# Megvii-CSG/MegReader

Hardware: AMD Instinct MI355X
Metric: training images/sec, CRNN-CTC 32x128 crops, batch 256 per GPU (higher is better)
Workload: dtype bf16; 1 GPU; CRNN + 1D-CTC training step (BASELINE.json configs[1]): 32x128 crops, T=33, C=38, Adam; global_batch=256, per_gpu_batch=256, parallelism=dp1, launch=hipGraph replay

## Files before the change

megreader_amd/csrc/igemm_core.h:

```cpp
#pragma once
#include "common.h"
#include <type_traits>

namespace mr {

struct ConvGeom {
  int Hg, Wg, Cg, ldg;
  int Hm, Wm;
  int R, S, sh, sw, ph, pw, dh, dw;
  int mode;
};

__device__ __forceinline__ bool conv_src(const ConvGeom& g, int hm, int wm, int r, int s, int& hi, int& wi) {
  if (g.mode == 1) {
    hi = hm * g.sh - g.ph + r * g.dh;
    wi = wm * g.sw - g.pw + s * g.dw;
  } else {
    int hn = hm + g.ph - r * g.dh;
    int wn = wm + g.pw - s * g.dw;
    if (hn < 0 || wn < 0) return false;
    if (g.sh == 1 && g.sw == 1) {
      hi = hn;
      wi = wn;
    } else {
      hi = hn / g.sh;
      wi = wn / g.sw;
      if (hi * g.sh != hn || wi * g.sw != wn) return false;
    }
  }
  return (unsigned)hi < (unsigned)g.Hg && (unsigned)wi < (unsigned)g.Wg;
}

template <typename T> struct Mma;
template <> struct Mma<bf16_t> {
  typedef bf16x8 Frag;
  static __device__ __forceinline__ void run(f32x4& acc, const Frag& a, const Frag& b) {
    acc = __builtin_amdgcn_mfma_f32_16x16x32_bf16(a, b, acc, 0, 0, 0);
  }
};
template <> struct Mma<float> {
  typedef f32x4 Frag;
  static __device__ __forceinline__ void run(f32x4& acc, const Frag& a, const Frag& b) {
#pragma unroll
    for (int j = 0; j < 4; ++j) acc = __builtin_amdgcn_mfma_f32_16x16x4f32(a[j], b[j], acc, 0, 0, 0);
  }
};

struct NtArgs {
  const void* A;
  const void* B;
  int M, N, K;
  long long lda;
  int ldb;
  const void* zero;
  int m_begin = 0;
  int ksplit = 1;
  void* ws = nullptr;
  int tile_rows = 0;
};
constexpr int NT_SPLIT_TICKETS = 4096;

__device__ __forceinline__ uint4 ldg16(const void* p) { return *(const uint4*)p; }

template <typename Epi> struct EpiHasStats { static constexpr bool value = false; };
template <typename Epi> struct EpiIsPool { static constexpr bool value = false; };
__device__ __forceinline__ float row16_sum(float v) {
#define MR_ROW_ROR(V, N) __builtin_bit_cast(float, __builtin_amdgcn_update_dpp(0, __builtin_bit_cast(int, V), 0x120 + (N), 0xf, 0xf, false))
  v += MR_ROW_ROR(v, 8);
  v += MR_ROW_ROR(v, 4);
  v += MR_ROW_ROR(v, 2);
  v += MR_ROW_ROR(v, 1);
#undef MR_ROW_ROR
  return v;
}
template <typename T, int CNT> struct EpiColStats {
  float s[4 * CNT], q[4 * CNT];
  __device__ __forceinline__ void init() {
#pragma unroll
    for (int e = 0; e < 4 * CNT; ++e) s[e] = q[e] = 0.f;
  }
  template <typename Epi> __device__ __forceinline__ void add(const Epi& epi, int m, int n, const f32x4* v) {
    if (m >= epi.M) return;
    if constexpr (Epi::kBnb) {
      const long long row = (long long)m * epi.ldc + n;
#pragma unroll
      for (int i = 0; i < CNT; ++i)
#pragma unroll
        for (int j = 0; j < 4; ++j) {
          const int c = 4 * i + j;
          if (n + c < epi.N) {
            float t = v[i][j];
            if (epi.addend) t += to_f32(epi.addend[row + c]);
            t = to_f32(from_f32<T>(t));
            if (epi.bnb_y && !(to_f32(epi.bnb_y[row + c]) > 0.f)) t = 0.f;
            s[c] += t;
            q[c] += t * to_f32(epi.bnb_x[row + c]);
          }
        }
    } else {
#pragma unroll
      for (int i = 0; i < CNT; ++i)
#pragma unroll
        for (int j = 0; j < 4; ++j) {
          float t = v[i][j];
          if (epi.bias && n + 4 * i + j < epi.N) t += epi.bias[n + 4 * i + j];
          t = to_f32(from_f32<T>(t));
          s[4 * i + j] += t;
          q[4 * i + j] += t * t;
        }
    }
  }
  template <typename Epi> __device__ __forceinline__ double q_out(const Epi& epi, int c, float sv, float qv) const {
    if constexpr (Epi::kBnb) return ((double)qv - (double)epi.bnb_mean[c] * (double)sv) * (double)epi.bnb_rstd[c];
    else return (double)qv;
  }
  template <typename Epi> __device__ __forceinline__ void flush(const Epi& epi, int n, int l15) {
#pragma unroll
    for (int e = 0; e < 4 * CNT; ++e) {
      s[e] = row16_sum(s[e]);
      q[e] = row16_sum(q[e]);
    }
    double* dst = epi.stats + (size_t)(blockIdx.x % epi.stats_ncopy) * 2 * epi.N;
    if constexpr (CNT == 4) {
      float sv = s[0], qv = q[0];
#pragma unroll
      for (int e = 1; e < 16; ++e) {
        sv = l15 == e ? s[e] : sv;
        qv = l15 == e ? q[e] : qv;
      }
      if (n + l15 < epi.N) {
        atomicAdd(dst + n + l15, (double)sv);
        atomicAdd(dst + epi.N + n + l15, q_out(epi, n + l15, sv, qv));
      }
    } else if constexpr (CNT == 2) {
      const int c = l15 & 7;
      float sv = s[0], qv = q[0];
#pragma unroll
      for (int e = 1; e < 8; ++e) {
        sv = c == e ? s[e] : sv;
        qv = c == e ? q[e] : qv;
      }
      if (n + c < epi.N) {
        if (l15 < 8) atomicAdd(dst + n + c, (double)sv);
        else atomicAdd(dst + epi.N + n + c, q_out(epi, n + c, sv, qv));
      }
    } else {
      if (l15 != 0) return;
#pragma unroll
      for (int e = 0; e < 4 * CNT; ++e)
        if (n + e < epi.N) {
          atomicAdd(dst + n + e, (double)s[e]);
          atomicAdd(dst + epi.N + n + e, q_out(epi, n + e, s[e], q[e]));
        }
    }
  }
};


template <typename T, int BM, int BN, int AMODE, typename Epi>
__device__ __forceinline__ void igemm_nt_body(const NtArgs& a, const ConvGeom& g, const Epi& epi) {
  constexpr int VEC = VecOf<T>::N;
  constexpr int BK = 8 * VEC;
  constexpr int AI = BM / 32, BI = BN / 32;
  constexpr int WTM = BM / 2, WTN = BN / 2, TM = WTM / 16, TN = WTN / 16;
  typedef typename Mma<T>::Frag Frag;

  __shared__ uint4 smem[8 * (BM + BN)];
  uint4* sA = smem;
  uint4* sB = smem + 8 * BM;

  const int tid = threadIdx.x;
  const int tiles_n = (a.N + BN - 1) / BN;
  const int tile_n = blockIdx.x % tiles_n, tile_m = blockIdx.x / tiles_n;
  const int m0 = tile_m * BM, n0 = tile_n * BN;
  const int kc = tid & 7, r0 = tid >> 3;

  const T* __restrict__ A = (const T*)a.A;
  const T* __restrict__ B = (const T*)a.B;

  long long a_off[AI];
  int a_h[AI], a_w[AI];
  unsigned a_mask[AI];
  bool a_ok[AI];
#pragma unroll
  for (int i = 0; i < AI; ++i) {
    const int m = m0 + r0 + 32 * i;
    a_ok[i] = m < a.M;
    a_mask[i] = 0;
    if (AMODE == 0) {
      a_off[i] = (long long)m * a.lda;
      a_h[i] = a_w[i] = 0;
    } else {
      const int wm = m % g.Wm;
      const int t = m / g.Wm;
      const int hm = t % g.Hm;
      const int ni = t / g.Hm;
      a_off[i] = (long long)ni * g.Hg * g.Wg * g.ldg;
      a_h[i] = hm;
      a_w[i] = wm;
      if (AMODE == 2) {
        const int bh = g.mode == 1 ? hm * g.sh - g.ph : hm + g.ph;
        const int bw = g.mode == 1 ? wm * g.sw - g.pw : wm + g.pw;
        a_off[i] += ((long long)bh * g.Wg + bw) * g.ldg;
        if (a_ok[i]) {
          unsigned msk = 0;
          for (int r = 0; r < g.R; ++r)
            for (int s2 = 0; s2 < g.S; ++s2) {
              int hi, wi;
              if (conv_src(g, hm, wm, r, s2, hi, wi)) msk |= 1u << (r * g.S + s2);
            }
          a_mask[i] = msk;
        }
      }
    }
  }
  long long b_off[BI];
  bool b_ok[BI];
#pragma unroll
  for (int i = 0; i < BI; ++i) {
    const int n = n0 + r0 + 32 * i;
    b_ok[i] = n < a.N;
    b_off[i] = (long long)n * a.ldb;
  }

  uint4 ra[AI], rb[BI];
  int f_tap = 0, f_r = 0, f_s = 0, f_c = kc * VEC;
  if (AMODE == 2) {
    while (f_c >= g.Cg) {
      f_c -= g.Cg;
      ++f_tap;
      if (++f_s == g.S) { f_s = 0; ++f_r; }
    }
  }
  const int taps = g.R * g.S;
  auto load_tiles = [&](int k0) {
    const int k = k0 + kc * VEC;
    const bool kok = k < a.K;
    int r = 0, s = 0, c = k;
    if (AMODE == 1) {
      const int tap = k / g.Cg;
      c = k - tap * g.Cg;
      r = tap / g.S;
      s = tap - r * g.S;
    }
    if (AMODE == 2) {
      const int toff = (f_r * g.dh * g.Wg + f_s * g.dw) * g.ldg;
      const long long koff = (long long)(g.mode == 1 ? toff : -toff) + f_c;
      const bool tok = f_tap < taps;
#pragma unroll
      for (int i = 0; i < AI; ++i) {
        uint4 v = make_uint4(0, 0, 0, 0);
        if (tok && ((a_mask[i] >> f_tap) & 1u)) v = ldg16(A + a_off[i] + koff);
        ra[i] = v;
      }
      f_c += BK;
      while (f_c >= g.Cg) {
        f_c -= g.Cg;
        ++f_tap;
        if (++f_s == g.S) { f_s = 0; ++f_r; }
      }
    } else {
#pragma unroll
      for (int i = 0; i < AI; ++i) {
        uint4 v = make_uint4(0, 0, 0, 0);
        if (a_ok[i] && kok) {
          if (AMODE == 0) {
            v = ldg16(A + a_off[i] + k);
          } else {
            int hi, wi;
            if (conv_src(g, a_h[i], a_w[i], r, s, hi, wi))
              v = ldg16(A + a_off[i] + ((long long)hi * g.Wg + wi) * g.ldg + c);
          }
        }
        ra[i] = v;
      }
    }
#pragma unroll
    for (int i = 0; i < BI; ++i) {
      uint4 v = make_uint4(0, 0, 0, 0);
      if (b_ok[i] && kok) v = ldg16(B + b_off[i] + k);
      rb[i] = v;
    }
  };

  const int wave = tid >> 6, lane = tid & 63;
  const int wm_ = wave & 1, wn_ = wave >> 1;
  const int l15 = lane & 15, lg = lane >> 4;

  f32x4 acc[TN][TM];
#pragma unroll
  for (int i = 0; i < TN; ++i)
#pragma unroll
    for (int j = 0; j < TM; ++j) acc[i][j] = (f32x4){0.f, 0.f, 0.f, 0.f};
  constexpr bool WIDE = sizeof(T) == 4;
  double tot[WIDE ? TN : 1][WIDE ? TM : 1][4];
  if constexpr (WIDE) {
#pragma unroll
    for (int i = 0; i < TN; ++i)
#pragma unroll
      for (int j = 0; j < TM; ++j)
#pragma unroll
        for (int e = 0; e < 4; ++e) tot[i][j][e] = 0.0;
  }

  load_tiles(0);
  for (int k0 = 0; k0 < a.K; k0 += BK) {
#pragma unroll
    for (int i = 0; i < AI; ++i) sA[kc * BM + ((r0 + 32 * i) ^ kc)] = ra[i];
#pragma unroll
// ... 356 lines not shown
#pragma unroll
    for (int i = 0; i < BI; ++i) {
      const bool ok = b_ok[i] && (k_exact || k0 + b_kc[i] < a.K);
      glds16_buf(rsB, ok, b_ptr[i] + k0, ESH, sB + (wave * BI + i) * 64);
    }
  };

  const int wm_ = wave & 1, wn_ = wave >> 1;
  const int l15 = lane & 15, lg = lane >> 4;
  const int xsw = (l15 >> 1) & 7;
  int fa_off[TM][2], fb_off[TN][2];
#pragma unroll
  for (int j = 0; j < TM; ++j) {
    const int r = wm_ * WTM + j * 16 + l15;
    fa_off[j][0] = r * 8 + (lg ^ xsw);
    fa_off[j][1] = r * 8 + ((lg ^ xsw) ^ 4);
  }
#pragma unroll
  for (int i = 0; i < TN; ++i) {
    const int r = wn_ * WTN + i * 16 + l15;
    fb_off[i][0] = BM * 8 + r * 8 + (lg ^ xsw);
    fb_off[i][1] = BM * 8 + r * 8 + ((lg ^ xsw) ^ 4);
  }

  f32x4 acc[TN][TM];
#pragma unroll
  for (int i = 0; i < TN; ++i)
#pragma unroll
    for (int j = 0; j < TM; ++j) acc[i][j] = (f32x4){0.f, 0.f, 0.f, 0.f};
  constexpr bool WIDE = sizeof(T) == 4;
  double tot[WIDE ? TN : 1][WIDE ? TM : 1][4];
  if constexpr (WIDE) {
#pragma unroll
    for (int i = 0; i < TN; ++i)
#pragma unroll
      for (int j = 0; j < TM; ++j)
#pragma unroll
        for (int e = 0; e < 4; ++e) tot[i][j][e] = 0.0;
  }

  auto compute = [&](const uint4* st) {
#pragma unroll
    for (int ks = 0; ks < 2; ++ks) {
      Frag fa[TM], fb[TN];
#pragma unroll
      for (int j = 0; j < TM; ++j) fa[j] = *(const Frag*)&st[fa_off[j][ks]];
#pragma unroll
      for (int i = 0; i < TN; ++i) fb[i] = *(const Frag*)&st[fb_off[i][ks]];
#pragma unroll
      for (int i = 0; i < TN; ++i)
#pragma unroll
        for (int j = 0; j < TM; ++j) Mma<T>::run(acc[i][j], fb[i], fa[j]);
    }
    if constexpr (WIDE) {
#pragma unroll
      for (int i = 0; i < TN; ++i)
#pragma unroll
        for (int j = 0; j < TM; ++j) {
#pragma unroll
          for (int e = 0; e < 4; ++e) tot[i][j][e] += (double)acc[i][j][e];
          acc[i][j] = (f32x4){0.f, 0.f, 0.f, 0.f};
        }
    }
  };

  const int nk_all = (a.K + BK - 1) / BK;
  int nk = nk_all, kb = 0;
  if (a.ksplit > 1) {
    const int per = (nk_all + a.ksplit - 1) / a.ksplit;
    const int first = (int)blockIdx.y * per;
    kb = first * BK;
    nk = min(per, nk_all - first);
    if (AMODE == 2) {
      s_tap = kb / g.Cg;
      s_c0 = kb - s_tap * g.Cg;
      s_r = s_tap / g.S;
      s_s = s_tap - s_r * g.S;
    }
  }
  if constexpr (NST == 2) {
    uint4* st0 = smem;
    uint4* st1 = smem + TILE_VECS;
    if (nk > 0) stage(st0, kb);
    int t = 0;
    for (; t + 1 < nk; t += 2) {
      __syncthreads();
      stage(st1, kb + (t + 1) * BK);
      compute(st0);
      __syncthreads();
      if (t + 2 < nk) stage(st0, kb + (t + 2) * BK);
      compute(st1);
    }
    if (t < nk) {
      __syncthreads();
      compute(st0);
    }
  } else {
    constexpr int LPS = AI + BI;
    static_assert((NST - 2) * LPS <= 63, "vmcnt is a 6-bit counter");
#pragma unroll
    for (int u = 0; u < NST - 1; ++u)
      if (u < nk) stage(smem + u * TILE_VECS, kb + u * BK);
    for (int t0 = 0; t0 < nk; t0 += NST) {
#pragma unroll
      for (int u = 0; u < NST; ++u) {
        const int t = t0 + u;
        if (t < nk) {
          const int younger = min(NST - 2, nk - 1 - t);
          if (younger >= 2 && NST >= 4) asm volatile("s_waitcnt vmcnt(%0)\n\ts_barrier" ::"n"(2 * LPS) : "memory");
          else if (younger == 1) asm volatile("s_waitcnt vmcnt(%0)\n\ts_barrier" ::"n"(LPS) : "memory");
          else asm volatile("s_waitcnt vmcnt(0)\n\ts_barrier" ::: "memory");
          if (t + NST - 1 < nk) stage(smem + ((u + NST - 1) % NST) * TILE_VECS, kb + (t + NST - 1) * BK);
          compute(smem + u * TILE_VECS);
        }
      }
    }
  }

  if constexpr (!WIDE) {
    if (a.ksplit > 1) {
      typedef __attribute__((ext_vector_type(4))) unsigned u32x4s;
      const int tile_lin = tile_m * tiles_n + tile_n;
      const rsrc_t rs = __builtin_amdgcn_make_buffer_rsrc((char*)a.ws + NT_SPLIT_TICKETS * 4, (short)0, 0x7fffffff, 0x00020000);
      constexpr int SLAB = BM * BN * 4;
      const int so = (tile_lin * a.ksplit + (int)blockIdx.y) * SLAB;
#pragma unroll
      for (int i = 0; i < TN; ++i)
#pragma unroll
        for (int j = 0; j < TM; ++j)
          __builtin_amdgcn_raw_buffer_store_b128(__builtin_bit_cast(u32x4s, acc[i][j]), rs, tid * 16, so + (i * TM + j) * 4096, 16);
      asm volatile("s_waitcnt vmcnt(0)" ::: "memory");
      __syncthreads();
      volatile int* bc = (volatile int*)smem;
      int* tk = (int*)a.ws + (tile_lin % NT_SPLIT_TICKETS);
      if (tid == 0) *bc = __hip_atomic_fetch_add(tk, 1, __ATOMIC_RELAXED, __HIP_MEMORY_SCOPE_AGENT);
      __syncthreads();
      if (*bc != a.ksplit - 1) return;
      if (tid == 0) __hip_atomic_store(tk, 0, __ATOMIC_RELAXED, __HIP_MEMORY_SCOPE_AGENT);
#pragma unroll
      for (int i = 0; i < TN; ++i)
#pragma unroll
        for (int j = 0; j < TM; ++j) acc[i][j] = (f32x4){0.f, 0.f, 0.f, 0.f};
      for (int sp = 0; sp < a.ksplit; ++sp) {
        const int sj = (tile_lin * a.ksplit + sp) * SLAB;
#pragma unroll
        for (int i = 0; i < TN; ++i)
#pragma unroll
          for (int j = 0; j < TM; ++j)
            acc[i][j] += __builtin_bit_cast(f32x4, __builtin_amdgcn_raw_buffer_load_b128(rs, tid * 16, sj + (i * TM + j) * 4096, 16));
      }
    }
  }

  EpiColStats<T, TN> cst;
  bool with_stats = false;
  if constexpr (EpiHasStats<Epi>::value) with_stats = epi.stats != nullptr;
  if (with_stats) cst.init();
#pragma unroll
  for (int j = 0; j < TM; ++j) {
    f32x4 run[TN];
#pragma unroll
    for (int i = 0; i < TN; ++i) {
      if constexpr (WIDE) run[i] = (f32x4){(float)tot[i][j][0], (float)tot[i][j][1], (float)tot[i][j][2], (float)tot[i][j][3]};
      else run[i] = acc[i][j];
    }
    if constexpr (EpiHasStats<Epi>::value)
      if (with_stats) cst.add(epi, m0 + wm_ * WTM + j * 16 + l15, n0 + wn_ * WTN + lg * (4 * TN), run);
    epi.template store_run<TN>(m0 + wm_ * WTM + j * 16 + l15, n0 + wn_ * WTN + lg * (4 * TN), run);
  }
  if constexpr (EpiHasStats<Epi>::value)
    if (with_stats) cst.flush(epi, n0 + wn_ * WTN + lg * (4 * TN), l15);
}

template <typename T, int WM, int WN, int TM, int TN, int AMODE, typename Epi>
__global__ __launch_bounds__(64 * WM * WN) void igemm_nt_big_kernel(NtArgs a, ConvGeom g, Epi epi) {
  constexpr int VEC = VecOf<T>::N;
  constexpr int BK = 8 * VEC;
  constexpr int NW = WM * WN;
  constexpr int WTM = TM * 16, WTN = TN * 16, BM = WM * WTM, BN = WN * WTN;
  constexpr int AG = BM / 8, BG = BN / 8;
  constexpr int AI = (AG + NW - 1) / NW, BI = (BG + NW - 1) / NW;
  constexpr int TILE_VECS = (BM + BN) * 8;
  typedef typename Mma<T>::Frag Frag;
  static_assert(AMODE == 0 || AMODE == 2, "big-tile kernel: dense or fast conv gather only");

  extern __shared__ uint4 smem_big[];
  uint4* smem = smem_big;

  const int tid = threadIdx.x;
  const int wave = __builtin_amdgcn_readfirstlane(tid >> 6);
  const int lane = tid & 63;
  const int trows = a.tile_rows > 0 ? a.tile_rows : BM;
  const int tiles_n = (a.N + BN - 1) / BN, tiles_m = (a.M - a.m_begin + trows - 1) / trows;
  const int xcd = blockIdx.x & 7, slot = blockIdx.x >> 3;
  const int tile_m = (slot / tiles_n) * 8 + xcd, tile_n = slot % tiles_n;
  if (tile_m >= tiles_m) return;
  const int m0 = a.m_begin + tile_m * trows, n0 = tile_n * BN;
  const int lrow = lane >> 3, lpc = lane & 7;

  const T* __restrict__ A = (const T*)a.A;
  const T* __restrict__ B = (const T*)a.B;
  (void)a.zero;
  constexpr int ESH = sizeof(T) == 2 ? 1 : 2;
  const rsrc_t rsA = make_rsrc(A), rsB = make_rsrc(B);

  auto kc_of = [&](int gi) { return (lpc ^ (((gi * 8 + lrow) >> 1) & 7)) * VEC; };
  int a_off[AI];
  unsigned a_mask[AI];
#pragma unroll
  for (int i = 0; i < AI; ++i) {
    const int gi = wave + i * NW;
    const int m = m0 + gi * 8 + lrow;
    a_mask[i] = 0;
    a_off[i] = 0;
    if (gi < AG && gi * 8 + lrow < trows) {
      if (AMODE == 0) {
        a_off[i] = (int)((long long)m * a.lda + kc_of(gi));
        a_mask[i] = m < a.M ? 1u : 0u;
      } else if (m < a.M) {
        const int wm = m % g.Wm;
        const int t = m / g.Wm;
        const int hm = t % g.Hm;
        const int ni = t / g.Hm;
        const int bh = g.mode == 1 ? hm * g.sh - g.ph : hm + g.ph;
        const int bw = g.mode == 1 ? wm * g.sw - g.pw : wm + g.pw;
        a_off[i] = (int)((long long)ni * g.Hg * g.Wg * g.ldg + ((long long)bh * g.Wg + bw) * g.ldg + kc_of(gi));
        unsigned msk = 0;
        for (int r = 0; r < g.R; ++r)
          for (int s2 = 0; s2 < g.S; ++s2) {
            int hi, wi;
            if (conv_src(g, hm, wm, r, s2, hi, wi)) msk |= 1u << (r * g.S + s2);
          }
        a_mask[i] = msk;
      }
    }
  }
  int b_off[BI];
  unsigned b_okmask = 0;
#pragma unroll
  for (int i = 0; i < BI; ++i) {
    const int gi = wave + i * NW;
    const int row = gi * 8 + lrow;
    const int rb = row % WTN;
    const int n = n0 + (row - rb) + ((rb >> 2) & 3) * (4 * TN) + (rb >> 4) * 4 + (rb & 3);
    if (gi < BG && n < a.N) b_okmask |= 1u << i;
    b_off[i] = (int)((long long)n * a.ldb + kc_of(gi));
  }

  const int sgn = g.mode == 1 ? 1 : -1;
  const bool k_exact = (a.K % BK) == 0;
  int s_tap = 0, s_r = 0, s_s = 0, s_c0 = 0;

  auto stage = [&](uint4* sA, int k0) {
    uint4* sB = sA + BM * 8;
    if (AMODE == 0) {
#pragma unroll
      for (int i = 0; i < AI; ++i) {
        const int gi = wave + i * NW;
        if (AG % NW == 0 || gi < AG) {
          const bool ok = a_mask[i] && (k_exact || k0 + kc_of(gi) < a.K);
          glds16_buf(rsA, ok, a_off[i] + k0, ESH, sA + gi * 64);
        }
      }
    } else {
      const int koff = sgn * ((s_r * g.dh * g.Wg + s_s * g.dw) * g.ldg) + s_c0;
      const unsigned bit = 1u << s_tap;
#pragma unroll
      for (int i = 0; i < AI; ++i) {
        const int gi = wave + i * NW;
        if (AG % NW == 0 || gi < AG) glds16_buf(rsA, a_mask[i] & bit, a_off[i] + koff, ESH, sA + gi * 64);
      }
      s_c0 += BK;
      if (s_c0 >= g.Cg) {
        s_c0 = 0;
        ++s_tap;
        if (++s_s == g.S) { s_s = 0; ++s_r; }
      }
    }
#pragma unroll
    for (int i = 0; i < BI; ++i) {
      const int gi = wave + i * NW;
      if (BG % NW == 0 || gi < BG) {
        const bool ok = ((b_okmask >> i) & 1u) && (k_exact || k0 + kc_of(gi) < a.K);
        glds16_buf(rsB, ok, b_off[i] + k0, ESH, sB + gi * 64);
      }
    }
  };

  const int wm_ = wave % WM, wn_ = wave / WM;
  const int l15 = lane & 15, lg = lane >> 4;
  const int xsw = (l15 >> 1) & 7;
  const int fa_base = (wm_ * WTM + l15) * 8 + (lg ^ xsw);
  const int fb_base = BM * 8 + (wn_ * WTN + l15) * 8 + (lg ^ xsw);

  f32x4 acc[TN][TM];
#pragma unroll
  for (int i = 0; i < TN; ++i)
#pragma unroll
    for (int j = 0; j < TM; ++j) acc[i][j] = (f32x4){0.f, 0.f, 0.f, 0.f};

  auto compute = [&](const uint4* st) {
#pragma unroll
    for (int ks = 0; ks < 2; ++ks) {
      const uint4* sa = st + (ks ? (fa_base ^ 4) : fa_base);
      const uint4* sb = st + (ks ? (fb_base ^ 4) : fb_base);
      Frag fb[TN];
#pragma unroll
      for (int i = 0; i < TN; ++i) fb[i] = *(const Frag*)&sb[i * 128];
      Frag fa = *(const Frag*)&sa[0];
#pragma unroll
      for (int j = 0; j < TM; ++j) {
        Frag nxt = fa;
        if (j + 1 < TM) nxt = *(const Frag*)&sa[(j + 1) * 128];
#pragma unroll
        for (int i = 0; i < TN; ++i) Mma<T>::run(acc[i][j], fb[i], fa);
        fa = nxt;
      }
    }
  };

  const int nk = (a.K + BK - 1) / BK;
  uint4* st0 = smem;
  uint4* st1 = smem + TILE_VECS;
  if (nk > 0) stage(st0, 0);
  int t = 0;
  for (; t + 1 < nk; t += 2) {
    __syncthreads();
    stage(st1, (t + 1) * BK);
    compute(st0);
    __syncthreads();
    if (t + 2 < nk) stage(st0, (t + 2) * BK);
    compute(st1);
  }
  if (t < nk) {
    __syncthreads();
    compute(st0);
  }

  if constexpr (EpiIsPool<Epi>::value) {
    static_assert(sizeof(T) == 2, "pooled epilogue: bf16 only");
    constexpr int CH = BN / 8;
    static_assert((CH & (CH - 1)) == 0 && (4 * TN) % 8 == 0, "pooled epilogue: tile width / lane run in whole 16-byte chunks");
    __syncthreads();
#pragma unroll
    for (int j = 0; j < TM; ++j) {
      const int r = wm_ * WTM + j * 16 + l15;
#pragma unroll
      for (int q = 0; q < TN / 2; ++q) {
        const int n = n0 + wn_ * WTN + lg * (4 * TN) + q * 8;
        T o[8];
#pragma unroll
        for (int e = 0; e < 8; ++e) {
          float t = acc[2 * q + e / 4][j][e % 4];
          if (epi.bias && n + e < epi.N) t += epi.bias[n + e];
          if (epi.relu) t = fmaxf(t, 0.f);
          o[e] = from_f32<T>(t);
        }
        const int c = (wn_ * WTN + lg * (4 * TN)) / 8 + q;
        smem[r * CH + (c ^ (r & (CH - 1)))] = *(const uint4*)o;
      }
    }
    __syncthreads();
    const int img_rows = trows / epi.Wo;
    const int prows = img_rows / epi.kh;
    const int row0 = m0 / epi.Wo;
    constexpr int PSTEP = 64 * NW / CH;
    const int c = tid % CH;
    int pix = tid / CH;
    int pr = pix / epi.PWo, pwi = pix - pr * epi.PWo;
    int nimg = (row0 + pr * epi.kh) / epi.Ho, h = (row0 + pr * epi.kh) - nimg * epi.Ho;
    const bool col_ok = n0 + c * 8 < epi.N;
    auto pool_one = [&](auto kh_tag, auto kw_tag) {
      constexpr int KH = decltype(kh_tag)::value, KW = decltype(kw_tag)::value;
      const int kh = KH ? KH : epi.kh, kw = KW ? KW : epi.kw;
      for (; pr < prows; ) {
        if (nimg < epi.Nimg && col_ok) {
          float best[8];
          unsigned char bi[8] = {0, 0, 0, 0, 0, 0, 0, 0};
#pragma unroll
          for (int e = 0; e < 8; ++e) best[e] = -INFINITY;
          bool first = true;
#pragma unroll
          for (int i = 0; i < (KH ? KH : 1); ++i)
            for (int i2 = 0; i2 < (KH ? 1 : kh); ++i2) {
              const int ii = KH ? i : i2;
#pragma unroll
              for (int jx = 0; jx < (KW ? KW : 1); ++jx)
                for (int j2 = 0; j2 < (KW ? 1 : kw); ++j2) {
                  const int jj = KW ? jx : j2;
                  const int w = pwi * epi.sw - epi.pw + jj;
                  if ((unsigned)w >= (unsigned)epi.Wo) continue;
                  const int r = (pr * kh + ii) * epi.Wo + w;
                  const uint4 v = smem[r * CH + (c ^ (r & (CH - 1)))];
                  const T* pv = (const T*)&v;
#pragma unroll
                  for (int e = 0; e < 8; ++e) {
                    const float f = to_f32(pv[e]);
                    if (first || f > best[e] || f != f) { best[e] = f; bi[e] = (unsigned char)(ii * kw + jj); }
                  }
                  first = false;
                }
            }
          T o[8];
#pragma unroll
          for (int e = 0; e < 8; ++e) o[e] = from_f32<T>(best[e]);
          const long long q = (((long long)nimg * epi.PHo + h / kh) * epi.PWo + pwi) * epi.ldc + n0 + c * 8;
          *(uint4*)(epi.C + q) = *(const uint4*)o;
          *(uint2*)(epi.idx + q) = *(const uint2*)bi;
        }
        pwi += PSTEP;
        while (pwi >= epi.PWo) {
          pwi -= epi.PWo;
          ++pr;
          h += kh;
          if (h >= epi.Ho) { h -= epi.Ho; ++nimg; }
        }
      }
    };
    if (epi.kh == 2 && epi.kw == 2) pool_one(std::integral_constant<int, 2>{}, std::integral_constant<int, 2>{});
    else pool_one(std::integral_constant<int, 0>{}, std::integral_constant<int, 0>{});
    return;
  } else {
  EpiColStats<T, TN> cst;
  bool with_stats = false;
  if constexpr (EpiHasStats<Epi>::value) with_stats = epi.stats != nullptr;
  if (with_stats) cst.init();
#pragma unroll
  for (int j = 0; j < TM; ++j) {
    f32x4 run[TN];
#pragma unroll
    for (int i = 0; i < TN; ++i) run[i] = acc[i][j];
    if constexpr (EpiHasStats<Epi>::value)
      if (with_stats) cst.add(epi, m0 + wm_ * WTM + j * 16 + l15, n0 + wn_ * WTN + lg * (4 * TN), run);
    epi.template store_run<TN>(m0 + wm_ * WTM + j * 16 + l15, n0 + wn_ * WTN + lg * (4 * TN), run);
  }
  if constexpr (EpiHasStats<Epi>::value)
    if (with_stats) cst.flush(epi, n0 + wn_ * WTN + lg * (4 * TN), l15);
  }
}

template <typename T> struct EpiPool {
  T* C;
  unsigned char* idx;
  long long ldc;
  const float* bias;
  int relu;
  int M, N;
  int Nimg, Ho, Wo, kh, kw, sw, pw, PHo, PWo;
};
template <typename T> struct EpiIsPool<EpiPool<T>> { static constexpr bool value = true; };

template <typename T> struct EpiStore {
  T* C;
  long long ldc;
  const float* bias;
  int relu;
  int M, N;
  int vec_ok;
  double* stats = nullptr;
  int stats_ncopy = 1;
  const T* addend = nullptr;
  static constexpr bool kBnb = false;
  __device__ __forceinline__ void operator()(int m, int n, f32x4 v) const {
    if (m >= M || n >= N) return;
    if (bias) {
#pragma unroll
      for (int j = 0; j < 4; ++j)
        if (n + j < N) v[j] += bias[n + j];
    }
    if (addend) {
      const T* a = addend + (long long)m * ldc + n;
#pragma unroll
      for (int j = 0; j < 4; ++j)
        if (n + j < N) v[j] += to_f32(a[j]);
    }
    if (relu) {
#pragma unroll
      for (int j = 0; j < 4; ++j) v[j] = fmaxf(v[j], 0.f);
    }
    T* p = C + (long long)m * ldc + n;
    if (vec_ok && n + 3 < N) {
      store4(p, v);
    } else {
#pragma unroll
      for (int j = 0; j < 4; ++j)
        if (n + j < N) p[j] = from_f32<T>(v[j]);
    }
  }
  template <int CNT>
  __device__ __forceinline__ void store_run(int m, int n, const f32x4* v) const {
    constexpr int E16 = 16 / (int)sizeof(T);
    if (m >= M) return;
    if (vec_ok && (ldc % E16) == 0 && (n % E16) == 0 && n + 4 * CNT <= N && (4 * CNT) % E16 == 0) {
      uint4* dst = (uint4*)(C + (long long)m * ldc + n);
      if (addend) {
        const uint4* asrc = (const uint4*)(addend + (long long)m * ldc + n);
#pragma unroll
        for (int q = 0; q < 4 * CNT / E16; ++q) {
          const uint4 av = asrc[q];
          const T* ap = (const T*)&av;
          T out[E16];
#pragma unroll
          for (int e = 0; e < E16; ++e) {
            const int c = q * E16 + e;
            float t = v[c / 4][c % 4] + to_f32(ap[e]);
            if (bias) t += bias[n + c];
            if (relu) t = fmaxf(t, 0.f);
            out[e] = from_f32<T>(t);
          }
          dst[q] = *(const uint4*)out;
        }
        return;
      }
      float x[4 * CNT];
#pragma unroll
      for (int i = 0; i < CNT; ++i)
#pragma unroll
        for (int j = 0; j < 4; ++j) {
          float t = v[i][j];
          if (bias) t += bias[n + 4 * i + j];
          if (relu) t = fmaxf(t, 0.f);
          x[4 * i + j] = t;
        }
      T out[4 * CNT];
#pragma unroll
      for (int e = 0; e < 4 * CNT; ++e) out[e] = from_f32<T>(x[e]);
      const uint4* src = (const uint4*)out;
#pragma unroll
      for (int q = 0; q < 4 * CNT / E16; ++q) dst[q] = src[q];
    } else {
#pragma unroll
      for (int i = 0; i < CNT; ++i) (*this)(m, n + 4 * i, v[i]);
    }
  }
};
template <typename T> struct EpiStoreB : EpiStore<T> {
  const T* bnb_x = nullptr;
  const T* bnb_y = nullptr;
  const float* bnb_mean = nullptr;
  const float* bnb_rstd = nullptr;
  static constexpr bool kBnb = true;
};
#ifndef MR_NO_EPI_STATS
template <typename T> struct EpiHasStats<EpiStore<T>> { static constexpr bool value = true; };
template <typename T> struct EpiHasStats<EpiStoreB<T>> { static constexpr bool value = true; };
#endif

struct TnArgs {
  const void* A;
  const void* B;
  float* C;
  int P, NA, NB;
  long long lda, ldb;
  int ldc;
  int p_chunk;
  int row_perm_h;
  float* colsum;
  float* colsum2 = nullptr;
  const int2* rowtab;
  int grp;
  void* ws;
  int fin = 0;
};
constexpr int TN_TICKETS = 4096;

static __global__ void tn_rowtab_kernel(ConvGeom g, int P, int2* __restrict__ tab) {
  const int p = blockIdx.x * blockDim.x + threadIdx.x;
  if (p >= P) return;
  const int qw = p % g.Wm;
  const int t = p / g.Wm;
  const int qh = t % g.Hm;
  const int qn = t / g.Hm;
  unsigned mask = 0;
  for (int r = 0; r < g.R; ++r)
    for (int s = 0; s < g.S; ++s) {
// ... 830 lines not shown
```

megreader_amd/csrc/igemm_p8.h:

```cpp
#pragma once
#include "igemm_core.h"

#ifndef MR_P8_SCHED
#define MR_P8_SCHED() __builtin_amdgcn_sched_barrier(0)
#endif

namespace mr {

template <int AMODE, typename Epi, int ABL = 0>
__global__ __launch_bounds__(512) void igemm_nt_p8_kernel(NtArgs a, ConvGeom g, Epi epi) {
  typedef bf16_t T;
  typedef Mma<T>::Frag Frag;
  constexpr int VEC = 8, BK = 64, BM = 256, BN = 256;
  constexpr int STAGE_VECS = (BM + BN) * 8;
  static_assert(AMODE == 0 || AMODE == 2, "phased kernel: dense or fast conv gather only");

  extern __shared__ uint4 smem_p8[];
  uint4* smem = smem_p8;

  const int tid = threadIdx.x;
  const int wave = __builtin_amdgcn_readfirstlane(tid >> 6);
  const int lane = tid & 63;
  const int tiles_n = (a.N + BN - 1) / BN, tiles_m = (a.M - a.m_begin + BM - 1) / BM;
  const int xcd = blockIdx.x & 7, slot = blockIdx.x >> 3;
// ... 34 lines not shown
        unsigned msk = 0;
        for (int r = 0; r < g.R; ++r)
          for (int s2 = 0; s2 < g.S; ++s2) {
            int hi, wi;
            if (conv_src(g, hm, wm, r, s2, hi, wi)) msk |= 1u << (r * g.S + s2);
          }
        a_mask[hh][j] = msk;
      }
      const int row = gi * 8 + lrow;
      const int rb = row % 64;
      const int n = n0 + (row - rb) + ((rb >> 2) & 3) * 16 + (rb >> 4) * 4 + (rb & 3);
      if (n < a.N) b_ok |= 1u << (hh * 2 + j);
      b_off[hh][j] = (int)((long long)n * a.ldb + kc_of(gi));
    }

  const int sgn = g.mode == 1 ? 1 : -1;
  const bool k_exact = (a.K % BK) == 0;
  const int nk = (a.K + BK - 1) / BK;
  int s_tap = 0, s_r = 0, s_s = 0, s_c0 = 0, s_ka = 0;

  auto stage_a = [&](int S, int hh) {
    uint4* dst = smem + S * STAGE_VECS;
    if (AMODE == 0) {
#pragma unroll
      for (int j = 0; j < 2; ++j) {
        const int gi = hh * 16 + wave + 8 * j;
        const bool ok = a_mask[hh][j] && (k_exact || s_ka + kc_of(gi) < a.K);
        glds16_buf(rsA, ok, a_off[hh][j] + s_ka, 1, dst + gi * 64);
      }
    } else {
      const int koff = sgn * ((s_r * g.dh * g.Wg + s_s * g.dw) * g.ldg) + s_c0;
      const unsigned bit = 1u << s_tap;
#pragma unroll
      for (int j = 0; j < 2; ++j) {
        const int gi = hh * 16 + wave + 8 * j;
        glds16_buf(rsA, a_mask[hh][j] & bit, a_off[hh][j] + koff, 1, dst + gi * 64);
      }
    }
  };
  auto advance_a = [&]() {
    if (AMODE == 0) {
      s_ka += BK;
    } else {
      s_c0 += BK;
      if (s_c0 >= g.Cg) {
        s_c0 = 0;
        ++s_tap;
        if (++s_s == g.S) { s_s = 0; ++s_r; }
      }
    }
  };
  auto stage_b = [&](int S, int hh, int k0) {
    uint4* dst = smem + S * STAGE_VECS + BM * 8;
#pragma unroll
    for (int j = 0; j < 2; ++j) {
      const int gi = hh * 16 + wave + 8 * j;
      const bool ok = ((b_ok >> (hh * 2 + j)) & 1u) && (k_exact || k0 + kc_of(gi) < a.K);
      glds16_buf(rsB, ok, b_off[hh][j] + k0, 1, dst + gi * 64);
    }
  };

  const int wm_ = wave & 1, wn_ = wave >> 1;
  const int l15 = lane & 15, lg = lane >> 4;
  const int xsw = (l15 >> 1) & 7;
  const int fa_base = (wm_ * 128 + l15) * 8 + (lg ^ xsw);
  const int fb_base = BM * 8 + (wn_ * 64 + l15) * 8 + (lg ^ xsw);

  f32x4 acc[4][8];
#pragma unroll
  for (int i = 0; i < 4; ++i)
#pragma unroll
    for (int j = 0; j < 8; ++j) acc[i][j] = (f32x4){0.f, 0.f, 0.f, 0.f};

  Frag fa0[4][2], fa1[4][2], fb0[2][2], fb1[2][2];
  auto read_a = [&](const uint4* st, int mh, Frag (&f)[4][2]) {
#pragma unroll
    for (int j = 0; j < 4; ++j)
#pragma unroll
      for (int ks = 0; ks < 2; ++ks) f[j][ks] = *(const Frag*)&st[(ks ? (fa_base ^ 4) : fa_base) + (mh * 4 + j) * 128];
  };
  auto read_b = [&](const uint4* st, int nh, Frag (&f)[2][2]) {
#pragma unroll
    for (int i = 0; i < 2; ++i)
#pragma unroll
      for (int ks = 0; ks < 2; ++ks) f[i][ks] = *(const Frag*)&st[(ks ? (fb_base ^ 4) : fb_base) + (nh * 2 + i) * 128];
  };
  auto mma_quad = [&](int mh, int nh, const Frag (&fa)[4][2], const Frag (&fb)[2][2]) {
#pragma unroll
    for (int ks = 0; ks < 2; ++ks)
#pragma unroll
      for (int i = 0; i < 2; ++i)
#pragma unroll
        for (int j = 0; j < 4; ++j) Mma<T>::run(acc[nh * 2 + i][mh * 4 + j], fb[i][ks], fa[j][ks]);
  };

  stage_b(0, 0, 0);
  stage_b(0, 1, 0);
  stage_a(0, 0);
  stage_a(0, 1);
  advance_a();
  if (nk > 1) {
    stage_a(1, 0);
    stage_a(1, 1);
    advance_a();
    asm volatile("s_waitcnt vmcnt(4)" ::: "memory");
  } else {
    asm volatile("s_waitcnt vmcnt(0)" ::: "memory");
  }
  __builtin_amdgcn_s_barrier();

  auto ktile = [&](int c, int S) {
    const uint4* st = smem + S * STAGE_VECS;
    const bool more1 = (ABL & 1) ? false : c + 1 < nk, more2 = (ABL & 1) ? false : c + 2 < nk;
    const bool rd = (ABL & 2) ? c == 0 : true;
    if (rd) {
    read_a(st, 0, fa0);
    read_b(st, 0, fb0);
    read_b(st, 1, fb1);
    }
    if (more1) stage_b(S ^ 1, 0, (c + 1) * BK);
    MR_P8_SCHED();
    mma_quad(0, 0, fa0, fb0);
    MR_P8_SCHED();
    if (rd) read_a(st, 1, fa1);
    if (more1) stage_b(S ^ 1, 1, (c + 1) * BK);
    MR_P8_SCHED();
    mma_quad(0, 1, fa0, fb1);
    MR_P8_SCHED();
    asm volatile("s_waitcnt lgkmcnt(0)" ::: "memory");
    __builtin_amdgcn_s_barrier();
    if (rd) read_b(st, 0, fb0);
    if (more2) stage_a(S, 0);
    MR_P8_SCHED();
    mma_quad(1, 1, fa1, fb1);
    MR_P8_SCHED();
    if (more2) { stage_a(S, 1); advance_a(); }
    MR_P8_SCHED();
    mma_quad(1, 0, fa1, fb0);
    MR_P8_SCHED();
    if (more2)
      asm volatile("s_waitcnt vmcnt(4)" ::: "memory");
    else
      asm volatile("s_waitcnt vmcnt(0)" ::: "memory");
    __builtin_amdgcn_s_barrier();
  };

  int c = 0;
  for (; c + 1 < nk; c += 2) {
    ktile(c, 0);
    ktile(c + 1, 1);
  }
  if (c < nk) ktile(c, 0);

  EpiColStats<bf16_t, 4> cst;
  bool with_stats = false;
  if constexpr (EpiHasStats<Epi>::value) with_stats = epi.stats != nullptr;
  if (with_stats) cst.init();
#pragma unroll
  for (int j = 0; j < 8; ++j) {
    f32x4 run[4];
#pragma unroll
    for (int i = 0; i < 4; ++i) run[i] = acc[i][j];
    if constexpr (EpiHasStats<Epi>::value)
      if (with_stats) cst.add(epi, m0 + wm_ * 128 + j * 16 + l15, n0 + wn_ * 64 + lg * 16, run);
    epi.template store_run<4>(m0 + wm_ * 128 + j * 16 + l15, n0 + wn_ * 64 + lg * 16, run);
  }
  if constexpr (EpiHasStats<Epi>::value)
    if (with_stats) cst.flush(epi, n0 + wn_ * 64 + lg * 16, l15);
}

}
```

Before: 104,900 images/s.

## Add specialized vectorized interior-tile epilogues for implicit-GEMM conv kernels

Adds a fast epilogue for wave tiles that lie fully inside the output. It is specialised at compile time on bias, relu, residual add, stats and BN-backward, and writes whole 16-byte vectors with bias and addend loads hoisted. It also prefetches the next row's addend and BN inputs, and uses sched barriers to pace loads and stores. The pooled epilogue is made bias/relu compile-time specialised as well. This removes per-element bounds checks and runtime branches in the epilogue, at the cost of more template instantiations, code size and register pressure.

```diff
diff --git a/megreader_amd/csrc/igemm_core.h b/megreader_amd/csrc/igemm_core.h
--- a/megreader_amd/csrc/igemm_core.h
+++ b/megreader_amd/csrc/igemm_core.h
@@ -155,6 +155,197 @@
     }
   }
 };
+
+__device__ __forceinline__ void pin_here(uint4& a) {
+  asm volatile("" : "+v"(a.x), "+v"(a.y), "+v"(a.z), "+v"(a.w));
+}
+template <typename T, int TM, int TN, bool BIAS, bool RELU, bool ADD, bool STATS, typename Epi, typename AccF>
+__device__ __forceinline__ void nt_store_interior(const Epi& epi, int m, int n, int l15, AccF&& acc_of) {
+  constexpr int E16 = 16 / (int)sizeof(T), NQ = 4 * TN / E16;
+  constexpr int VARIANT = (int)BIAS | (int)RELU << 1 | (int)ADD << 2 | (int)STATS << 3;
+  float bv[4 * TN];
+  if constexpr (BIAS) {
+    const float* __restrict__ bp = epi.bias + n;
+#pragma unroll
+    for (int c = 0; c < 4 * TN; ++c) bv[c] = bp[c];
+  }
+  EpiColStats<T, TN> cst;
+  if constexpr (STATS) cst.init();
+  const long long row0 = (long long)m * epi.ldc + n;
+  const long long rstep = 16 * epi.ldc / E16;
+  uint4* dst = (uint4*)(epi.C + row0);
+  const uint4* asrc = nullptr;
+  uint4 av[NQ];
+  if constexpr (ADD) {
+    asrc = (const uint4*)(epi.addend + row0);
+#pragma unroll
+    for (int q = 0; q < NQ; ++q) av[q] = asrc[q];
+  }
+#pragma unroll
+  for (int j = 0; j < TM; ++j) {
+    uint4 out[NQ];
+#pragma unroll
+    for (int q = 0; q < NQ; ++q) {
+      f32x4 v[E16 / 4];
+#pragma unroll
+      for (int i = 0; i < E16 / 4; ++i) {
+        v[i] = acc_of(q * (E16 / 4) + i, j);
+        asm volatile("; nt epilogue variant %1" : "+v"(v[i]) : "n"(VARIANT));
+      }
+      if constexpr (ADD) pin_here(av[q]);
+      T o[E16];
+#pragma unroll
+      for (int e = 0; e < E16; ++e) {
+        const int c = q * E16 + e;
+        float t = v[e / 4][e % 4];
+        if constexpr (ADD) t += to_f32(((const T*)&av[q])[e]);
+        if constexpr (BIAS) t += bv[c];
+        if constexpr (STATS) {
+          const float r = to_f32(from_f32<T>(t));
+          cst.s[c] += r;
+          cst.q[c] += r * r;
+        }
+        if constexpr (RELU) t = fmaxf(t, 0.f);
+        o[e] = from_f32<T>(t);
+      }
+      out[q] = *(const uint4*)o;
+      __builtin_amdgcn_sched_barrier(0);
+    }
+    if constexpr (ADD) {
+      __builtin_amdgcn_sched_barrier(0);
+      if (j + 1 < TM) {
+        asrc += rstep;
+#pragma unroll
+        for (int q = 0; q < NQ; ++q) av[q] = asrc[q];
+      }
+    }
+    __builtin_amdgcn_sched_barrier(0);
+#pragma unroll
+    for (int q = 0; q < NQ; ++q) dst[q] = out[q];
+    dst += rstep;
+    __builtin_amdgcn_sched_barrier(0);
+  }
+  if constexpr (STATS) cst.flush(epi, n, l15);
+}
+
+template <typename T, int TM, int TN, bool ADD, bool HASY, typename Epi, typename AccF>
+__device__ __forceinline__ void nt_store_interior_bnb(const Epi& epi, int m, int n, int l15, AccF&& acc_of) {
+  constexpr int E16 = 16 / (int)sizeof(T), NQ = 4 * TN / E16;
+  constexpr int VARIANT = 16 | (int)ADD | (int)HASY << 1;
+  EpiColStats<T, TN> cst;
+  cst.init();
+  const long long row0 = (long long)m * epi.ldc + n;
+  const long long rstep = 16 * epi.ldc / E16;
+  uint4* dst = (uint4*)(epi.C + row0);
+  const uint4* xsrc = (const uint4*)(epi.bnb_x + row0);
+  const uint4* ysrc = HASY ? (const uint4*)(epi.bnb_y + row0) : nullptr;
+  const uint4* asrc = ADD ? (const uint4*)(epi.addend + row0) : nullptr;
+  uint4 xv[NQ], yv[NQ], av[NQ];
+#pragma unroll
+  for (int q = 0; q < NQ; ++q) {
+    xv[q] = xsrc[q];
+    if constexpr (HASY) yv[q] = ysrc[q];
+    if constexpr (ADD) av[q] = asrc[q];
+  }
+#pragma unroll
+  for (int j = 0; j < TM; ++j) {
+    uint4 out[NQ];
+#pragma unroll
+    for (int q = 0; q < NQ; ++q) {
+      f32x4 v[E16 / 4];
+#pragma unroll
+      for (int i = 0; i < E16 / 4; ++i) {
+        v[i] = acc_of(q * (E16 / 4) + i, j);
+        asm volatile("; nt epilogue variant %1" : "+v"(v[i]) : "n"(VARIANT));
+      }
+      pin_here(xv[q]);
+      if constexpr (HASY) pin_here(yv[q]);
+      if constexpr (ADD) pin_here(av[q]);
+      T o[E16];
+#pragma unroll
+      for (int e = 0; e < E16; ++e) {
+        const int c = q * E16 + e;
+        float t = v[e / 4][e % 4];
+        if constexpr (ADD) t += to_f32(((const T*)&av[q])[e]);
+        o[e] = from_f32<T>(t);
+        float r = to_f32(o[e]);
+        if constexpr (HASY)
+          if (!(to_f32(((const T*)&yv[q])[e]) > 0.f)) r = 0.f;
+        cst.s[c] += r;
+        cst.q[c] += r * to_f32(((const T*)&xv[q])[e]);
+      }
+      out[q] = *(const uint4*)o;
+      __builtin_amdgcn_sched_barrier(0);
+    }
+    __builtin_amdgcn_sched_barrier(0);
+    if (j + 1 < TM) {
+      xsrc += rstep;
+      if constexpr (HASY) ysrc += rstep;
+      if constexpr (ADD) asrc += rstep;
+#pragma unroll
+      for (int q = 0; q < NQ; ++q) {
+        xv[q] = xsrc[q];
+        if constexpr (HASY) yv[q] = ysrc[q];
+        if constexpr (ADD) av[q] = asrc[q];
+      }
+    }
+    __builtin_amdgcn_sched_barrier(0);
+#pragma unroll
+    for (int q = 0; q < NQ; ++q) dst[q] = out[q];
+    dst += rstep;
+    __builtin_amdgcn_sched_barrier(0);
+  }
+  cst.flush(epi, n, l15);
+}
+
+constexpr int NT_EPI_PLAIN = 1, NT_EPI_ADD = 2, NT_EPI_STATS = 4, NT_EPI_BNB = 8;
+constexpr int NT_EPI_STORE = NT_EPI_PLAIN | NT_EPI_ADD | NT_EPI_STATS;
+template <typename T, int TM, int TN, int PATHS, typename Epi, typename AccF>
+__device__ __forceinline__ bool nt_epilogue_interior(const Epi& epi, int wave_m0, int wave_n0, int l15, int lg, AccF&& acc_of) {
+  constexpr int E16 = 16 / (int)sizeof(T);
+  const int m = wave_m0 + l15, n = wave_n0 + lg * (4 * TN);
+  bool with_stats = false;
+  if constexpr (EpiHasStats<Epi>::value) with_stats = epi.stats != nullptr;
+  if constexpr ((4 * TN) % E16 == 0) {
+    const bool interior = epi.vec_ok && (epi.ldc % E16) == 0 && wave_m0 + 16 * TM <= epi.M && wave_n0 + 16 * TN <= epi.N;
+    const bool has_bias = epi.bias != nullptr, has_add = epi.addend != nullptr;
+    if constexpr (Epi::kBnb) {
+      const bool xy_vec = (((uintptr_t)epi.bnb_x | (uintptr_t)epi.bnb_y) & 15) == 0;
+      if ((PATHS & NT_EPI_BNB) && interior && xy_vec && with_stats && !has_bias && !epi.relu) {
+        const bool has_y = epi.bnb_y != nullptr;
+        if (has_add) {
+          if (has_y) nt_store_interior_bnb<T, TM, TN, true, true>(epi, m, n, l15, acc_of);
+          else nt_store_interior_bnb<T, TM, TN, true, false>(epi, m, n, l15, acc_of);
+        } else {
+          if (has_y) nt_store_interior_bnb<T, TM, TN, false, true>(epi, m, n, l15, acc_of);
+          else nt_store_interior_bnb<T, TM, TN, false, false>(epi, m, n, l15, acc_of);
+        }
+        return true;
+      }
+    } else if (interior && !(with_stats && has_add) && (PATHS & (has_add ? NT_EPI_ADD : with_stats ? NT_EPI_STATS : NT_EPI_PLAIN))) {
+      auto go = [&](auto bias_tag, auto relu_tag) {
+        constexpr bool B = decltype(bias_tag)::value, R = decltype(relu_tag)::value;
+        if (has_add) {
+          if constexpr ((PATHS & NT_EPI_ADD) != 0) nt_store_interior<T, TM, TN, B, R, true, false>(epi, m, n, l15, acc_of);
+        } else if (with_stats) {
+          if constexpr ((PATHS & NT_EPI_STATS) != 0 && EpiHasStats<Epi>::value)
+            nt_store_interior<T, TM, TN, B, R, false, true>(epi, m, n, l15, acc_of);
+        } else {
+          if constexpr ((PATHS & NT_EPI_PLAIN) != 0) nt_store_interior<T, TM, TN, B, R, false, false>(epi, m, n, l15, acc_of);
+        }
+      };
+      if (has_bias) {
+        if (epi.relu) go(std::true_type{}, std::true_type{});
+        else go(std::true_type{}, std::false_type{});
+      } else {
+        if (epi.relu) go(std::false_type{}, std::true_type{});
+        else go(std::false_type{}, std::false_type{});
+      }
+      return true;
+    }
+  }
+  return false;
+}
 
 
 template <typename T, int BM, int BN, int AMODE, typename Epi>
@@ -817,6 +1008,17 @@
     }
   }
 
+  constexpr int EPI_PATHS = Epi::kBnb ? ((sizeof(T) == 2 && NST == 2) ? NT_EPI_BNB : 0)
+                            : NST != 2 ? (BM >= 96 ? (NT_EPI_PLAIN | NT_EPI_ADD) : 0)
+                            : sizeof(T) == 2 ? (NT_EPI_PLAIN | NT_EPI_ADD | ((BM == 64 && BN == 128) ? 0 : NT_EPI_STATS))
+                                             : (NT_EPI_PLAIN | (BM == 128 ? (NT_EPI_ADD | NT_EPI_STATS) : 0));
+  if constexpr (EPI_PATHS != 0) {
+    if (nt_epilogue_interior<T, TM, TN, EPI_PATHS>(epi, m0 + wm_ * WTM, n0 + wn_ * WTN, l15, lg, [&](int i, int j) -> f32x4 {
+          if constexpr (WIDE) return (f32x4){(float)tot[i][j][0], (float)tot[i][j][1], (float)tot[i][j][2], (float)tot[i][j][3]};
+          else return acc[i][j];
+        }))
+      return;
+  }
   EpiColStats<T, TN> cst;
   bool with_stats = false;
   if constexpr (EpiHasStats<Epi>::value) with_stats = epi.stats != nullptr;
@@ -1007,23 +1209,38 @@
     constexpr int CH = BN / 8;
     static_assert((CH & (CH - 1)) == 0 && (4 * TN) % 8 == 0, "pooled epilogue: tile width / lane run in whole 16-byte chunks");
     __syncthreads();
-#pragma unroll
-    for (int j = 0; j < TM; ++j) {
-      const int r = wm_ * WTM + j * 16 + l15;
-#pragma unroll
-      for (int q = 0; q < TN / 2; ++q) {
-        const int n = n0 + wn_ * WTN + lg * (4 * TN) + q * 8;
-        T o[8];
-#pragma unroll
-        for (int e = 0; e < 8; ++e) {
-          float t = acc[2 * q + e / 4][j][e % 4];
-          if (epi.bias && n + e < epi.N) t += epi.bias[n + e];
-          if (epi.relu) t = fmaxf(t, 0.f);
-          o[e] = from_f32<T>(t);
-        }
-        const int c = (wn_ * WTN + lg * (4 * TN)) / 8 + q;
-        smem[r * CH + (c ^ (r & (CH - 1)))] = *(const uint4*)o;
-      }
+    auto tile_to_lds = [&](auto bias_tag, auto relu_tag) {
+      constexpr bool BIAS = decltype(bias_tag)::value, RELU = decltype(relu_tag)::value;
+      const int nl = n0 + wn_ * WTN + lg * (4 * TN);
+      float bv[4 * TN];
+      if constexpr (BIAS) {
+#pragma unroll
+        for (int e = 0; e < 4 * TN; ++e) bv[e] = nl + e < epi.N ? epi.bias[nl + e] : 0.f;
+      }
+#pragma unroll
+      for (int j = 0; j < TM; ++j) {
+        const int r = wm_ * WTM + j * 16 + l15;
+#pragma unroll
+        for (int q = 0; q < TN / 2; ++q) {
+          T o[8];
+#pragma unroll
+          for (int e = 0; e < 8; ++e) {
+            float t = acc[2 * q + e / 4][j][e % 4];
+            if constexpr (BIAS) t += bv[q * 8 + e];
+            if constexpr (RELU) t = fmaxf(t, 0.f);
+            o[e] = from_f32<T>(t);
+          }
+          const int c = (wn_ * WTN + lg * (4 * TN)) / 8 + q;
+          smem[r * CH + (c ^ (r & (CH - 1)))] = *(const uint4*)o;
+        }
+      }
+    };
+    if (epi.bias != nullptr) {
+      if (epi.relu) tile_to_lds(std::true_type{}, std::true_type{});
+      else tile_to_lds(std::true_type{}, std::false_type{});
+    } else {
+      if (epi.relu) tile_to_lds(std::false_type{}, std::true_type{});
+      else tile_to_lds(std::false_type{}, std::false_type{});
     }
     __syncthreads();
     const int img_rows = trows / epi.Wo;
@@ -1086,6 +1303,13 @@
     else pool_one(std::integral_constant<int, 0>{}, std::integral_constant<int, 0>{});
     return;
   } else {
+    constexpr bool FLAGSHIP = (WM == 2 && WN == 4 && TM == 8 && TN == 4) || (WM == 1 && WN == 8 && TM == 17 && TN == 2);
+    constexpr int EPI_PATHS = FLAGSHIP ? NT_EPI_STORE : (TN == 2 && !(WM == 4 && TM == 3)) ? (NT_EPI_PLAIN | NT_EPI_ADD) : 0;
+    if constexpr (EPI_PATHS != 0) {
+      if (nt_epilogue_interior<T, TM, TN, EPI_PATHS>(epi, m0 + wm_ * WTM, n0 + wn_ * WTN, l15, lg,
+                                                      [&](int i, int j) -> f32x4 { return acc[i][j]; }))
+        return;
+    }
   EpiColStats<T, TN> cst;
   bool with_stats = false;
   if constexpr (EpiHasStats<Epi>::value) with_stats = epi.stats != nullptr;
diff --git a/megreader_amd/csrc/igemm_p8.h b/megreader_amd/csrc/igemm_p8.h
--- a/megreader_amd/csrc/igemm_p8.h
+++ b/megreader_amd/csrc/igemm_p8.h
@@ -210,6 +210,9 @@
   }
   if (c < nk) ktile(c, 0);
 
+  if (nt_epilogue_interior<bf16_t, 8, 4, NT_EPI_STORE>(epi, m0 + wm_ * 128, n0 + wn_ * 64, l15, lg,
+                                                      [&](int i, int j) -> f32x4 { return acc[i][j]; }))
+    return;
   EpiColStats<bf16_t, 4> cst;
   bool with_stats = false;
   if constexpr (EpiHasStats<Epi>::value) with_stats = epi.stats != nullptr;
```

New measurement: 109,100 images/s (median of 6 runs). +4.0%, better.
